# PhilippBongartz/RepeatResolver

Measured on AMD Instinct MI355X. Metric: sum-of-pairs DP cells/sec, higher is better.
Workload: dtype u32

## Files before the change

include/pwr.h:

```cpp
#ifndef PWR_H
#define PWR_H

#include <stddef.h>
#include <stdint.h>
#include <stdio.h>

#ifdef __cplusplus
extern "C" {
#endif

#define PWR_OK 0
#define PWR_ERR_ARG (-1)
#define PWR_ERR_NOMEM (-2)
#define PWR_ERR_DEVICE (-3)
#define PWR_ERR_INPUT (-4)
#define PWR_ERR_RANGE (-5)
#define PWR_ERR_INTERNAL (-6)
#define PWR_ERR_UNSUPPORTED (-7)
#define PWR_ERR_IO (-8)
#define PWR_ERR_STALL (-9)
#define PWR_ERR_ORDER (-10)

#define PWR_MAX_BANDWIDTH 2000
#define PWR_MAX_SEQ_LENGTH 35000
// ... 21 lines not shown
    uint64_t rows_jumped;
} pwr_stats;

int pwr_create(pwr_ctx **out, int rows, int width, const unsigned char *text, int bandwidth, int device);
void pwr_destroy(pwr_ctx *ctx);

int pwr_trim_ends(pwr_ctx *ctx);
int pwr_realign_row(pwr_ctx *ctx, int k);
int pwr_realign_round(pwr_ctx *ctx);
int pwr_realign_rows(pwr_ctx *ctx, int k0, int n);
int pwr_split_begin(pwr_ctx *ctx, int k0, int n, int rank, int world);
int pwr_split_slot_bytes(pwr_ctx *ctx, size_t *slot_bytes, int *slots_per_rank);
int pwr_split_stage(pwr_ctx *ctx, void *send_dev);
int pwr_split_commit(pwr_ctx *ctx, const void *recv_dev, int *rows_left);
int pwr_total_score(pwr_ctx *ctx, uint64_t *total);
int pwr_dims(pwr_ctx *ctx, int *rows, int *width);
int pwr_export_rows(pwr_ctx *ctx, unsigned char *buf, size_t cap);
typedef struct pwr_snapshot pwr_snapshot;
int pwr_snapshot_begin(pwr_ctx *ctx, pwr_snapshot **snap);
int pwr_snapshot_wait(pwr_snapshot *snap, const unsigned char **image, size_t *bytes, int *rows, int *width);
void pwr_snapshot_free(pwr_snapshot *snap);

int pwr_set_option(pwr_ctx *ctx, const char *key, long value);
int pwr_get_option(pwr_ctx *ctx, const char *key, long *value);
int pwr_get_stats(pwr_ctx *ctx, pwr_stats *out);
int pwr_reset_stats(pwr_ctx *ctx);
const char *pwr_strerror(int code);
int pwr_device_count(void);

int pwr_read_msa_file(const char *path, int *rows, int *width, unsigned char **text, char *err, size_t errcap);
int pwr_write_msa_file(const char *path, int rows, int width, const unsigned char *text);
int pwr_run_file(const char *in_path, const char *out_path, int bandwidth, int device, int max_rounds, FILE *log);

#ifdef __cplusplus
}
#endif
#endif
```

repeatresolver_amd/_lib.py:

```python
import ctypes
import os

_HERE = os.path.dirname(os.path.abspath(__file__))
LIB_PATH = os.path.join(_HERE, "csrc", "libpwr.so")


class PwrStats(ctypes.Structure):
    _fields_ = [("cells_reference", ctypes.c_uint64), ("cells_computed", ctypes.c_uint64),
                ("fill_launches", ctypes.c_uint64), ("fill_ms", ctypes.c_double),
                ("rows_committed", ctypes.c_uint64), ("rows_recomputed", ctypes.c_uint64),
                ("batches", ctypes.c_uint64), ("rows_changed", ctypes.c_uint64),
                ("reject_reason", ctypes.c_uint64 * 4), ("fill_launches_timed", ctypes.c_uint64),
                ("stalls", ctypes.c_uint64), ("rows_ahead", ctypes.c_uint64), ("rows_wide", ctypes.c_uint64),
                ("seg_jobs", ctypes.c_uint64), ("segs", ctypes.c_uint64), ("seg_fails", ctypes.c_uint64),
                ("rows_jumped", ctypes.c_uint64)]


EXPORTS = ["pwr_create", "pwr_destroy", "pwr_trim_ends", "pwr_realign_row", "pwr_realign_round", "pwr_realign_rows",
           "pwr_total_score", "pwr_dims", "pwr_export_rows", "pwr_set_option", "pwr_get_option", "pwr_get_stats",
           "pwr_reset_stats", "pwr_strerror", "pwr_device_count", "pwr_read_msa_file",
           "pwr_write_msa_file", "pwr_run_file", "pwr_split_begin", "pwr_split_slot_bytes", "pwr_split_stage", "pwr_split_commit",
           "pwr_snapshot_begin", "pwr_snapshot_wait", "pwr_snapshot_free"]

PIA_EXPORTS = ["pia_create", "pia_destroy", "pia_align", "pia_get_stats", "pia_set_option", "pia_get_timing", "pia_read_template", "pia_read_fasta",
               "pia_build_msa", "pia_run_files"]

PRC_EXPORTS = ["prc_create", "prc_destroy", "prc_occurrences", "prc_cut", "prc_get_stats", "prc_free", "prc_read_template",
               "prc_read_fasta", "prc_scan_dense", "prc_scan_runs", "prc_select_cuts", "prc_write_seq", "prc_write_info",
               "prc_run_files"]

PMC_EXPORTS = ["pmc_maxcorrs", "pmc_last_timing", "pmc_read_msa", "pmc_write", "pmc_run_file"]

PGR_EXPORTS = ["pgr_refine", "pgr_free", "pgr_last_timing", "pgr_read_window", "pgr_window_free", "pgr_slice_maxcorrs",
               "pgr_read_maxcorrs_file", "pgr_default_cutoff", "pgr_restrict_coverage", "pgr_subdivide", "pgr_subdivision_free",
               "pgr_last_subdivision_timing", "pgr_dropoff_subdivision", "pgr_compress_labels", "pgr_complete_labels",
               "pgr_write_subdivision", "pgr_subdivision_name", "pgr_kmeans_subdivide", "pgr_kmeans_free", "pgr_kmeans_subdivide_pairs",
               "pgr_last_kmeans_timing", "pgr_kmeans_reassign", "pgr_msa_open", "pgr_msa_close", "pgr_msa_window", "pgr_msa_resolve",
               "pgr_resolution_free", "pgr_last_resolve_timing", "pgr_connect", "pgr_connection_free"]


class PgrWindow(ctypes.Structure):
    _fields_ = [("rows", ctypes.c_int), ("kept_rows", ctypes.c_int), ("von", ctypes.c_int), ("bis", ctypes.c_int),
                ("width", ctypes.c_int), ("sc", ctypes.c_int), ("kept", ctypes.POINTER(ctypes.c_ubyte)),
                ("groups", ctypes.POINTER(ctypes.c_uint64)), ("local_coverage", ctypes.POINTER(ctypes.c_uint64)),
                ("coverage", ctypes.POINTER(ctypes.c_int))]


class PgrResult(ctypes.Structure):
    _fields_ = [("rows", ctypes.c_int), ("kept_rows", ctypes.c_int), ("width", ctypes.c_int), ("sc", ctypes.c_int),
                ("nsig", ctypes.c_int), ("cutoff", ctypes.c_double), ("kept", ctypes.POINTER(ctypes.c_ubyte)),
                ("maxcorrs", ctypes.POINTER(ctypes.c_double)), ("significant", ctypes.POINTER(ctypes.c_int)),
                ("sizes", ctypes.POINTER(ctypes.c_int)), ("cliques", ctypes.POINTER(ctypes.c_int)),
                ("cutoffs", ctypes.POINTER(ctypes.c_int)), ("drop_off", ctypes.POINTER(ctypes.c_double)),
                ("c_groups", ctypes.POINTER(ctypes.c_uint64)), ("c_coverage", ctypes.POINTER(ctypes.c_uint64))]

# ... 70 lines not shown
    lib.pwr_export_rows.argtypes = [vp, ctypes.c_char_p, ctypes.c_size_t]
    lib.pwr_set_option.restype = ci
    lib.pwr_set_option.argtypes = [vp, ctypes.c_char_p, ctypes.c_long]
    lib.pwr_get_option.restype = ci
    lib.pwr_get_option.argtypes = [vp, ctypes.c_char_p, ctypes.POINTER(ctypes.c_long)]
    lib.pwr_get_stats.restype = ci
    lib.pwr_get_stats.argtypes = [vp, ctypes.POINTER(PwrStats)]
    lib.pwr_strerror.restype = ctypes.c_char_p
    lib.pwr_strerror.argtypes = [ci]
    lib.pwr_device_count.restype = ci
    lib.pwr_device_count.argtypes = []
    lib.pwr_split_begin.restype = ci
    lib.pwr_split_begin.argtypes = [vp, ci, ci, ci, ci]
    lib.pwr_split_slot_bytes.restype = ci
    lib.pwr_split_slot_bytes.argtypes = [vp, ctypes.POINTER(ctypes.c_size_t), ctypes.POINTER(ci)]
    lib.pwr_split_stage.restype = ci
    lib.pwr_split_stage.argtypes = [vp, vp]
    lib.pwr_split_commit.restype = ci
    lib.pwr_split_commit.argtypes = [vp, vp, ctypes.POINTER(ci)]
    if hasattr(lib, "pwr_snapshot_begin"):
        lib.pwr_snapshot_begin.restype = ci
        lib.pwr_snapshot_begin.argtypes = [vp, ctypes.POINTER(vp)]
        lib.pwr_snapshot_wait.restype = ci
        lib.pwr_snapshot_wait.argtypes = [vp, ctypes.POINTER(vp), ctypes.POINTER(ctypes.c_size_t), ctypes.POINTER(ci), ctypes.POINTER(ci)]
        lib.pwr_snapshot_free.restype = None
        lib.pwr_snapshot_free.argtypes = [vp]
    lib.pwr_debug_last_job.restype = ci
    lib.pwr_debug_last_job.argtypes = [vp, ctypes.POINTER(ci), ctypes.POINTER(ci), ctypes.POINTER(ci),
                                       ctypes.POINTER(ci), ctypes.POINTER(ci), ci]
    lib.pwr_debug_fill_clock.restype = ci
    lib.pwr_debug_fill_clock.argtypes = [vp, ctypes.POINTER(ctypes.c_double), ctypes.POINTER(ctypes.c_double)]
    lib.pwr_debug_row_columns.restype = ci
    lib.pwr_debug_row_columns.argtypes = [vp, ci, ctypes.POINTER(ci), ci]
    lib.pwr_debug_rounds.restype = ci
    lib.pwr_debug_rounds.argtypes = [vp]
    ll = ctypes.c_longlong
    lib.pia_create.restype = ci
    lib.pia_create.argtypes = [ctypes.POINTER(vp), ctypes.c_char_p, ci, ci]
    lib.pia_destroy.restype = None
    lib.pia_destroy.argtypes = [vp]
    lib.pia_align.restype = ci
    lib.pia_align.argtypes = [vp, ci, ctypes.c_char_p, ctypes.POINTER(ll), ctypes.POINTER(ci), ctypes.POINTER(ci)]
    lib.pia_get_stats.restype = ci
    lib.pia_get_stats.argtypes = [vp, ctypes.POINTER(ctypes.c_uint64), ctypes.POINTER(ctypes.c_double)]
    lib.pia_set_option.restype = ci
    lib.pia_set_option.argtypes = [vp, ctypes.c_char_p, ll]
    lib.pia_get_timing.restype = ci
    lib.pia_get_timing.argtypes = [vp, ctypes.POINTER(ctypes.c_double)]
    lib.pia_read_template.restype = ci
    lib.pia_read_template.argtypes = [ctypes.c_char_p, ctypes.POINTER(ctypes.c_void_p), ctypes.POINTER(ci)]
    lib.pia_read_fasta.restype = ci
    lib.pia_read_fasta.argtypes = [ctypes.c_char_p, ctypes.POINTER(ci), ctypes.POINTER(ctypes.c_void_p), ctypes.POINTER(ctypes.c_void_p)]
    lib.pia_build_msa.restype = ci
    lib.pia_build_msa.argtypes = [ctypes.c_char_p, ctypes.c_char_p, ci, ctypes.c_char_p, ctypes.POINTER(ll), ctypes.POINTER(ci),
                                  ctypes.POINTER(ci), ctypes.c_double, ci]
    lib.pmc_maxcorrs.restype = ci
    lib.pmc_maxcorrs.argtypes = [ci, ci, ctypes.c_char_p, ci, ci, ctypes.POINTER(ctypes.c_double)]
    lib.pmc_last_timing.restype = ci
    lib.pmc_last_timing.argtypes = [ctypes.POINTER(ctypes.c_double)]
    lib.pmc_read_msa.restype = ci
    lib.pmc_read_msa.argtypes = [ctypes.c_char_p, ctypes.POINTER(ci), ctypes.POINTER(ci), ctypes.POINTER(ctypes.c_void_p)]
    lib.pmc_write.restype = ci
    lib.pmc_write.argtypes = [ctypes.c_char_p, ci, ctypes.POINTER(ctypes.c_double)]
    pi, pll, cp = ctypes.POINTER(ci), ctypes.POINTER(ll), ctypes.c_char_p
    lib.prc_create.restype = ci
    lib.prc_create.argtypes = [ctypes.POINTER(vp), cp, ci, ci]
# ... 90 lines not shown
```

repeatresolver_amd/csrc/pwr_device.hip:

```cpp
#include <hip/hip_runtime.h>

#include <algorithm>
#include <chrono>
#include <cstdint>
#include <cstdio>
#include <cstdlib>
#include <cstring>
#include <new>
#include <thread>
#include <type_traits>
#include <vector>

#include "pwr.h"

#define PWR_INF 0x40000000u
#define PWR_BIG 0x7fffffff

struct Hdr {
    int W;
    int nslots;
    int nfree;
    int cur;
    int status;
    int stop;
// ... 108 lines not shown
    uint4 *desc;
    int wpNW, wpMS;
    unsigned *lastM;
    unsigned long long *gmb;
    SegDesc *seg;
    unsigned *chk;
    int seg_align;
    int src_start;
    int smax, seg_rows, warm_cols;
    int seg_budget, seg_minrows;
    int seg_balance;
    int plan_ahead;
    int hard_rows, hard_up, hard_down;
    int plan_len;
    int plan_gate_rel;
    int spec_inorder;
    int fail_stops;
    int plan_slack, plan_evrate_x100;
    const int *rowids;
    int gstride;
    unsigned tagbase;
    unsigned long long *gtr;
    int trk;
    unsigned trace_tag;
    long long *g64;
    int force64;
    int evcap;
    int gate_v2;
    int *chkdone;
    int check_in_trace, trace_ny;
    int trace_blk;
    int v2_follows, f64_follows;
    int stall_test;
    unsigned long long *diag;
    int njobs_launched;
    int Lmax, colcap, NC;
    size_t dirstride;
    int split_rank, split_world;
    CommitJob *cjob;
    int *chg;
    int *evkey, *evdl;
    int *insidx;
    int *pair_cf, *pair_left;
    BatchPlan *plan;
    CommitEv *sev;
    int *freed;
    unsigned *ticket;
};
#define NOT_MINE(JB, JOB) ((JB).split_world > 1 && (JOB) % (JB).split_world != (JB).split_rank)

#define DPP_ROW_SHR(n) (0x110 + (n))
#define DPP_ROW_BCAST15 0x142
#define DPP_ROW_BCAST31 0x143
#define DPP_WAVE_SHR1 0x138

__device__ __forceinline__ int wave_incl_min(int v)
{
    int t;
    t = __builtin_amdgcn_update_dpp(PWR_BIG, v, DPP_ROW_SHR(1), 0xF, 0xF, false); v = min(v, t);
    t = __builtin_amdgcn_update_dpp(PWR_BIG, v, DPP_ROW_SHR(2), 0xF, 0xF, false); v = min(v, t);
    t = __builtin_amdgcn_update_dpp(PWR_BIG, v, DPP_ROW_SHR(4), 0xF, 0xF, false); v = min(v, t);
    t = __builtin_amdgcn_update_dpp(PWR_BIG, v, DPP_ROW_SHR(8), 0xF, 0xF, false); v = min(v, t);
    t = __builtin_amdgcn_update_dpp(PWR_BIG, v, DPP_ROW_BCAST15, 0xA, 0xF, false); v = min(v, t);
    t = __builtin_amdgcn_update_dpp(PWR_BIG, v, DPP_ROW_BCAST31, 0xC, 0xF, false); v = min(v, t);
    return v;
}
// ... 858 lines not shown
        atomicAdd(&st.hdr->cells_computed, m->cells);
    }
#undef MBP
#undef MBM
#undef PTB
#undef LD64
#undef LD32LO
#undef ST64
}

#ifndef PWR_INTERIOR_CLS
#define PWR_INTERIOR_CLS 0
#endif
#define V3_TICKS() ((unsigned)(__builtin_amdgcn_s_memtime() >> 10))
#define V3_TIMEOUT_TICKS (1u << 19)
#define V4_RB 128

#ifdef PWR_DIAG
#define DG_DECL unsigned long long dg_wait_fast = 0, dg_wait_gen = 0, dg_wait_setup = 0, dg_t = 0, dg_t2 = 0, dg_cyc_int = 0, dg_cyc_gen16 = 0, dg_ts1 = 0, dg_ts2 = 0, dg_tl2 = 0; unsigned dg_log = 0; unsigned dg_int = 0, dg_gen16 = 0, dg_general = 0, dg_nowork = 0, dg_runs = 0, dg_switch = 0;
#define DG_T0() dg_t = __builtin_amdgcn_s_memtime();
#define DG_ADD(ACC) ACC += __builtin_amdgcn_s_memtime() - dg_t;
#define DG_INC(CNT, N) CNT += (N);
#define DG_T2() dg_t2 = __builtin_amdgcn_s_memtime();
#define DG_ADD2(ACC) ACC += __builtin_amdgcn_s_memtime() - dg_t2;
#else
#define DG_T2()
#define DG_ADD2(ACC)
#define DG_DECL
#define DG_T0()
#define DG_ADD(ACC)
#define DG_INC(CNT, N)
#endif
template <int NW, int C, bool WG1>
__global__ __launch_bounds__(WG1 ? NW * 64 : 128) void k_fill_v3(DState st, JobBufs jb)
{
    constexpr int MS = 64 * C, RS = NW * MS;
    constexpr int NL = WG1 ? NW : 1;
    constexpr int RB = WG1 ? 64 : V4_RB;
    __shared__ __attribute__((aligned(16))) int ldsS1[NL][2][4][MS];
    __shared__ unsigned long long rP[NL][RB], rM[NL][RB];
    __shared__ int wprog[NL], wdone;
    const int vjob = WG1 ? (int)blockIdx.x : (int)(blockIdx.x + 8 * blockIdx.z), lane = threadIdx.x & 63;
    const int role = WG1 ? 0 : UNI((int)threadIdx.x >> 6);
    const int wave = WG1 ? UNI((int)threadIdx.x >> 6) : (int)blockIdx.y;
    const int lw = WG1 ? wave : 0, wr = WG1 ? (wave + 1) % NW : 0;
    if (vjob >= jb.njobs_launched * jb.smax) return;
    const int job = vjob / jb.smax;
    const SegDesc *const sd = jb.seg + (size_t)job * SEG_MAX + (vjob % jb.smax);
    JobMeta *m = &jb.meta[job];
    if (st.hdr->fallback > 0 && jb.v2_follows) return;
    if (!m->active || m->L <= 0 || !m->ok || m->wide || !sd->active || NOT_MINE(jb, job)) return;
    const int seg_xb = UNI(sd->xb), seg_fin = UNI(sd->fin);
    const int L = UNI(sd->xe) - seg_xb;
    const int Lf = seg_fin ? L - 1 : L;
    const int x_own = UNI(sd->xown) - seg_xb;
    const int g_own = x_own >> 4;
    const int chkA = x_own > 0 ? x_own : -1, chkB = seg_fin ? -1 : L;
    unsigned *const chk_w = jb.chk + (((size_t)job * (SEG_MAX + 1) + sd->s) * 2 + 0) * (size_t)jb.NC;
    unsigned *const chk_t = jb.chk + (((size_t)job * (SEG_MAX + 1) + sd->s + 1) * 2 + 1) * (size_t)jb.NC;
    const unsigned long long t_clk0 = __builtin_amdgcn_s_memtime(), t_real0 = __builtin_amdgcn_s_memrealtime();
    for (int i = threadIdx.x; i < NL * RB; i += blockDim.x) { (&rP[0][0])[i] = 0; (&rM[0][0])[i] = 0; }
    if (threadIdx.x < NL) wprog[threadIdx.x] = 0;
    if (threadIdx.x == 0) wdone = 0;
    __syncthreads();

    const int wl = (wave + NW - 1) % NW;
    const unsigned tagbase = jb.tagbase;
    const size_t gstride = (size_t)jb.gstride;
    unsigned long long *const gmy = jb.gmb + (((size_t)job * NW + wave) * gstride + (size_t)sd->grow0) * 2;
    const unsigned long long *const gleftw = jb.gmb + (((size_t)job * NW + wl) * gstride + (size_t)sd->grow0) * 2;
    const unsigned long long *const gjob = jb.gmb + ((size_t)job * NW * gstride + (size_t)sd->grow0) * 2;
#define PTOT_PTR(AP, BP, R) (gjob + (((size_t)((((AP) + (BP) - 1 - lo) / MS) % NW)) * gstride + (size_t)(R)) * 2)
    int *const abortf = &m->abort;
#define GLD(PTR) __hip_atomic_load((PTR), __ATOMIC_RELAXED, __HIP_MEMORY_SCOPE_AGENT)
#define GST(PTR, VAL, ROW) __hip_atomic_store((PTR), ((unsigned long long)(tagbase | (unsigned)((ROW) + 1)) << 32) | (unsigned)(VAL), __ATOMIC_RELAXED, __HIP_MEMORY_SCOPE_AGENT)
#define GST2(PTR, VAL, TAG) __hip_atomic_store((PTR), ((unsigned long long)(TAG) << 32) | (unsigned)(VAL), __ATOMIC_RELAXED, __HIP_MEMORY_SCOPE_AGENT)
#define TAGOF(W64) ((unsigned)((W64) >> 32))
#define LLD(REF) __hip_atomic_load(&(REF), __ATOMIC_RELAXED, __HIP_MEMORY_SCOPE_WORKGROUP)
#define LST(REF, V) __hip_atomic_store(&(REF), (V), __ATOMIC_RELAXED, __HIP_MEMORY_SCOPE_WORKGROUP)

    if (!WG1 && role == 1) {
        for (unsigned it = 0;; ++it) {
            if (UNI(LLD(wdone))) break;
            const int wx = UNI(LLD(wprog[lw]));
            const int r = wx - 1 + lane;
            const bool inr = r >= 0 && r < L;
            unsigned long long p = 0, q = 0;
            int ab = 0;
            if (inr) { p = GLD(gleftw + 2 * (size_t)r); q = GLD(gleftw + 2 * (size_t)r + 1); }
            if ((it & 15u) == 15u) ab = GLD(abortf);
            if (inr) {
                const unsigned tagr = tagbase | (unsigned)(r + 1);
                if (TAGOF(p) == tagr && TAGOF(q) == tagr) {
                    LST(rP[lw][r & (RB - 1)], p);
                    __hip_atomic_store(&rM[lw][r & (RB - 1)], q, __ATOMIC_RELEASE, __HIP_MEMORY_SCOPE_WORKGROUP);
                }
            }
            if (UNI(ab)) break;
        }
        return;
    }

    const int lo = UNI(m->lo), hi = UNI(m->hi), W = UNI(m->W), B = st.B, H = st.H;
    const int *way = jb.way + (size_t)job * jb.Lmax + seg_xb;
    const uint8_t *seq = st.seq + st.rowoff[UNI(m->k)] + seg_xb;
    const int4 *rec2 = jb.rec2 + (size_t)job * jb.colcap * 2;
    uint32_t *dirs = jb.dirs + (size_t)job * jb.dirstride + (size_t)(seg_xb >> 4) * RS;
    unsigned *lastM = jb.lastM + (size_t)job * jb.NC;
    const int lc = lane * C;
#define V4_LOADS(MSX, SLOT, AU, AG, AI, GL)                                                      \
    {                                                                                            \
        const int yq_ = lo + (MSX) * MS - 1;                                                     \
        GL = (yq_ >= lo && yq_ <= hi) ? UNI(rec2[2 * (yq_ - lo) + 1].y) : 0;                     \
        int4 p_[C];                                                                              \
        _Pragma("unroll") for (int i = 0; i < C; ++i) {                                          \
            const int y_ = lo + (MSX) * MS + lc + i;                                             \
// ... 52 lines not shown
        _Pragma("unroll") for (int i = 0; i < C; ++i) { accA[i] <<= sh_; accC[i] <<= sh_; }      \
        nacc = (WANT);                                                                           \
    }
#define V4_FLUSH()                                                                               \
    if (gacc >= 0) {                                                                             \
        V4_ALIGN_ACC(16)                                                                         \
        uint32_t *d_ = dirs + (size_t)gacc * RS + (size_t)wave * MS + (size_t)lc;                \
        _Pragma("unroll") for (int i = 0; i < C; ++i) { if (gacc >= g_own) d_[i] = accA[i] | (accC[i] << 16); accA[i] = accC[i] = 0; } \
        gacc = -1; nacc = 0;                                                                     \
    }
#define V4_ROTATE_BLOCK()                                                                        \
    {                                                                                            \
        blk = x >> 6;                                                                            \
        wcur = wnxt; scur = snxt; dca = dna; dcf = dnf >> fsh;     \
        wnxt = way[min(x + 64 + lane, L - 1)];                                                   \
        snxt = seq[min(x + 64 + lane, L - 1)];                                                   \
        dna = desc[min(x + 64 + lane, L - 1)].x; dnf = descw[4 * min(x + 64 + lane, L - 1)];     \
    }
#define V4_NEXT_ROW()                                                                            \
    {                                                                                            \
        a_prev = a; Bx_prev = Bx;                                                                \
        ++x;                                                                                     \
        if (lane == 0) LST(wprog[lw], x);                                                            \
        if (x < L) {                                                                             \
            if ((x >> 6) != blk) V4_ROTATE_BLOCK()                                               \
            a = max(0, __builtin_amdgcn_readlane(wcur, x & 63) - H);                             \
            sx = __builtin_amdgcn_readlane(scur, x & 63);                                        \
        }                                                                                        \
    }

    DG_DECL
#ifdef PWR_DIAG
    unsigned long long *const tl = jb.diag + ((size_t)job * 32 + 31) * 4096 + (size_t)(sd->s * NW + wave) * 6;
    if (lane == 0 && sd->s * NW + wave < 680) { tl[0] = t_real0; tl[1] = __builtin_amdgcn_s_memrealtime(); tl[2] = 0; }
#endif
#define V4_EARLY_MASKS()                                                                         \
    if (early_hi >= (blk << 6)) {                                                                \
        const int b0_ = blk << 6;                                                                \
        const int lo_ = max(early_lo, b0_) - b0_, hi_ = min(early_hi, b0_ + 64) - b0_;           \
        const unsigned long long me_ = hi_ > lo_ ? ((hi_ - lo_ >= 64 ? ~0ull : ((1ull << (hi_ - lo_)) - 1ull)) << lo_) : 0ull; \
        const unsigned long long mf_ = early_hi < b0_ + 64 ? 1ull << (early_hi - b0_) : 0ull;    \
        bOm |= me_ | mf_; bMm |= me_ | mf_; bPm |= me_; bTm |= me_;                              \
    }
    bool dead = jb.stall_test && vjob == 0 && wave == 0;
    int first_pending = 0;
    int early_lo = 0, early_hi = -1;
    while (x < L && !dead) {
        ran_prev = UNI(ran_prev); gacc = UNI(gacc); nacc = UNI(nacc); blk = UNI(blk); ms = UNI(ms); cs = UNI(cs); gleft = UNI(gleft);
        x = UNI(x);
#ifdef PWR_DIAG
        if (ran_prev && !dg_tl2) { dg_tl2 = __builtin_amdgcn_s_memrealtime(); if (lane == 0 && sd->s * NW + wave < 680) { tl[2] = dg_tl2; tl[5] = (unsigned long long)x; } }
#endif
        if ((ran_prev || first_pending) && x < Lf) {
            unsigned long long bOm = __builtin_amdgcn_ballot_w64((dcf & 1u) != 0);
            const bool first = UNI(first_pending) != 0;
            if (first || ((bOm >> (x & 63)) & 1ull)) {
                first_pending = 0;
                unsigned long long bPm = __builtin_amdgcn_ballot_w64((dcf & 2u) != 0);
                unsigned long long bMm = __builtin_amdgcn_ballot_w64((dcf & 4u) != 0);
                unsigned long long bTm = __builtin_amdgcn_ballot_w64((dcf & 8u) != 0);
                if (first) { bOm |= 1ull << (x & 63); bMm |= 1ull << (x & 63); }
                V4_EARLY_MASKS()
                int dcaf = (int)(dca & 0xffffffu), dcb = min(dcaf + B, W);
                unsigned dcs = min(dca >> 24, 3u) * (unsigned)(MS * 4);
                if ((x >> 4) != gacc) { V4_FLUSH() gacc = x >> 4; }
                V4_ALIGN_ACC(x & 15)
                if (lane == 0) LST(wprog[lw], x);
                unsigned mlast_v = 0;
                if (first) {
                    const unsigned tagp = tagbase | (unsigned)x;
                    const int yq = lo + ms * MS - 1;
                    const bool needM = yq >= a_prev && yq < a_prev + Bx_prev;
                    unsigned long long eT = 0, eM = 0;
                    DG_T0()
#ifdef PWR_DIAG
                    const unsigned long long ev_t0 = __builtin_amdgcn_s_memrealtime();
#endif
                    const unsigned t0 = V3_TICKS();
                    for (unsigned spin = 1;; ++spin) {
                        eT = GLD(PTOT_PTR(a_prev, Bx_prev, x - 1));
                        eM = LLD(rM[lw][(x - 1) & (RB - 1)]);
                        if (UNI(TAGOF(eT)) == tagp && (!needM || UNI(TAGOF(eM)) == tagp)) break;
                        if ((spin & 1023u) == 0 && (V3_TICKS() - t0 > V3_TIMEOUT_TICKS || UNI(GLD(abortf)))) { dead = true; break; }
                        __builtin_amdgcn_s_sleep(1);
// ... 407 lines not shown
            const unsigned left0 = (unsigned)__builtin_amdgcn_update_dpp((int)mrow, (int)Mn[C - 1], DPP_WAVE_SHR1, 0xF, 0xF, false);
#pragma unroll
            for (int i = 0; i < C; ++i) {
                const unsigned lf = i ? Mn[i > 0 ? i - 1 : 0] : left0;
                const bool inb = (unsigned)(rel0 + i) < (unsigned)Bx;
                accA[i] = (accA[i] << 1) | ((((fa >> i) & 1u) || (inb && Mn[i] == lf)) ? 1u : 0u);
                lastM[wave * MS + lc + i] = inb ? Mn[i] : 0xffffffffu;
            }
        }
        nacc = (x & 15) + 1;
        if (lane == 63) {
            GST(gmy + 2 * (size_t)x, P_end, x);
            if (WG1) {
                const unsigned long long tg_ = (unsigned long long)(tagbase | (unsigned)(x + 1)) << 32;
                LST(rP[wr][x & (RB - 1)], tg_ | (unsigned)P_end);
                LST(rM[wr][x & (RB - 1)], tg_ | (unsigned)Mprev[C - 1]);
            } else GST(gmy + 2 * (size_t)x + 1, Mprev[C - 1], x);
        }
        ran_prev = 1;
        V4_CHK_STORE(x + 1, a, a + Bx)
        V4_NEXT_ROW()
    }
    V4_FLUSH()
#ifdef PWR_DIAG
    if (lane == 0) {
        unsigned long long *dgp = jb.diag + ((size_t)job * 32 + wave) * 4096;
        dgp[0] = __builtin_amdgcn_s_memtime() - t_clk0; dgp[1] = dg_wait_fast; dgp[2] = dg_wait_gen; dgp[3] = dg_wait_setup;
        dgp[4] = ((unsigned long long)dg_int << 32) | dg_gen16; dgp[5] = ((unsigned long long)dg_general << 32) | dg_nowork;
        dgp[6] = ((unsigned long long)dg_runs << 32) | dg_switch; dgp[7] = (unsigned long long)L;
        dgp[12] = dg_log; dgp[8] = dg_cyc_gen16; dgp[9] = dg_ts1; dgp[10] = dg_ts2; dgp[11] = dg_cyc_int;
    }
#endif
#ifdef PWR_DIAG
    if (lane == 0 && sd->s * NW + wave < 680) { tl[3] = __builtin_amdgcn_s_memrealtime(); tl[4] = (unsigned long long)L | ((unsigned long long)(dg_wait_fast + dg_wait_gen + dg_wait_setup) << 20); }
#endif
    if (lane == 0) { LST(wprog[lw], 0x7fffffff); LST(wdone, 1); }
    if (dead) {
        if (lane == 0) __hip_atomic_store(abortf, 1, __ATOMIC_RELAXED, __HIP_MEMORY_SCOPE_AGENT);
        return;
    }
    if (wave == 0 && lane == 0) {
        if (sd->s == 0) {
            m->clk = (unsigned)(__builtin_amdgcn_s_memtime() - t_clk0);
            m->rclk = (unsigned)(__builtin_amdgcn_s_memrealtime() - t_real0);
            m->rounds = 0;
        }
        atomicAdd(&st.hdr->cells_computed, sd->cells);
    }
#undef V4_CHK_STORE
#undef V4_EARLY_MASKS
#undef PTOT_PTR
#undef GLD
#undef GST
#undef GST2
#undef TAGOF
#undef LLD
#undef LST
#undef V4_LOADS
#undef V4_ALIGN_ACC
#undef V4_FLUSH
#undef V4_ROTATE_BLOCK
#undef V4_NEXT_ROW
}

__device__ __forceinline__ bool seg_check_applies(const DState &st, const JobBufs &jb, int job, const JobMeta *m)
{
    return m->active && m->L > 0 && m->ok && !m->wide && !m->abort && !(st.hdr->fallback > 0 && jb.v2_follows) && !NOT_MINE(jb, job) && m->nseg > 1;
}

// ... 2207 lines not shown
    if ((rc = regrow(c, &st.inscnt, 0, ncap))) return rc;
    if ((rc = regrow(c, &st.newidx, 0, ncap))) return rc;
    st.colcap = (int)ncap; st.slotcap = (int)ncap;
    const int nj = c->njobs;
    free_jobs(c);
    if ((rc = alloc_jobs(c, nj))) return rc;
    const int zero = 0;
    HIPC(hipMemcpy(&st.hdr->need_grow, &zero, sizeof(int), hipMemcpyHostToDevice));
    return PWR_OK;
}

static int launch_fill(pwr_ctx *c, int njobs)
{
    hipEvent_t e0 = nullptr, e1 = nullptr;
    const bool timed = c->profile && (c->stats.fill_launches % (unsigned)c->profile) == 0 && c->ev_used < (size_t)(1 << 16);
    if (timed) {
        if (c->ev_used == c->ev_pool.size()) {
            hipEvent_t a, b;
            HIPC(hipEventCreate(&a)); HIPC(hipEventCreate(&b));
            c->ev_pool.emplace_back(a, b);
        }
        e0 = c->ev_pool[c->ev_used].first; e1 = c->ev_pool[c->ev_used].second;
        c->ev_used++;
        HIPC(hipEventRecord(e0, c->stream));
    }
    if (c->fill_mode == 4) {
        if (++c->fill_epoch >= (1u << 15)) {
            const size_t nmb = (size_t)c->njobs * c->wp_waves * c->jb.gstride * 2;
            HIPC(hipMemsetAsync(c->jb.gmb, 0, nmb * 8, c->stream));
            c->fill_epoch = 1;
        }
        c->jb.tagbase = c->fill_epoch << 17;
        c->jb.njobs_launched = njobs;
        c->jb.stall_test = c->stall_test > 0 ? 1 : 0;
        c->jb.v2_follows = (c->seen_fallback > 0 && c->wp_waves != 17) ? 1 : 0;
        if (c->stall_test > 0) c->stall_test -= 1;
        const int nv = njobs * c->jb.smax;
        const dim3 grid(8, c->wp_waves, (nv + 7) / 8);
        const bool wg1 = c->one_wg && c->wp_waves <= 9 && c->B <= 1024 && c->wave_cols != 4;
        if (wg1) {
            const size_t pad = (size_t)c->one_wg_lds;
            if (c->wp_waves == 5) hipLaunchKernelGGL((k_fill_v3<5, 4, true>), dim3(nv), dim3(5 * 64), pad, c->stream, c->st, c->jb);
            else if (c->wp_waves == 8) hipLaunchKernelGGL((k_fill_v3<8, 3, true>), dim3(nv), dim3(8 * 64), pad, c->stream, c->st, c->jb);
            else if (c->wp_waves == 4) hipLaunchKernelGGL((k_fill_v3<4, 6, true>), dim3(nv), dim3(4 * 64), pad, c->stream, c->st, c->jb);
            else if (c->wp_waves == 3) hipLaunchKernelGGL((k_fill_v3<3, 8, true>), dim3(nv), dim3(3 * 64), pad, c->stream, c->st, c->jb);
            else hipLaunchKernelGGL((k_fill_v3<9, 2, true>), dim3(nv), dim3(9 * 64), pad, c->stream, c->st, c->jb);
        }
        else if (c->wp_waves == 17) hipLaunchKernelGGL((k_fill_v3<17, 1, false>), grid, dim3(128), 0, c->stream, c->st, c->jb);
        else if (c->wp_waves == 5) hipLaunchKernelGGL((k_fill_v3<5, 4, false>), grid, dim3(128), (size_t)c->fill_lds, c->stream, c->st, c->jb);
        else if (c->wp_waves == 8) hipLaunchKernelGGL((k_fill_v3<8, 3, false>), grid, dim3(128), 0, c->stream, c->st, c->jb);
        else if (c->wp_waves == 4) hipLaunchKernelGGL((k_fill_v3<4, 6, false>), grid, dim3(128), 0, c->stream, c->st, c->jb);
        else if (c->wp_waves == 3) hipLaunchKernelGGL((k_fill_v3<3, 8, false>), grid, dim3(128), 0, c->stream, c->st, c->jb);
        else if (c->B <= 1024 && c->wave_cols != 4) hipLaunchKernelGGL((k_fill_v3<9, 2, false>), grid, dim3(128), 0, c->stream, c->st, c->jb);
        else hipLaunchKernelGGL((k_fill_v3<9, 4, false>), grid, dim3(128), 0, c->stream, c->st, c->jb);
        c->jb.stall_test = 0;
        if (c->jb.smax > 1 && c->jb.seg_rows > 0 && !c->jb.check_in_trace)
            hipLaunchKernelGGL(k_seg_check, dim3(njobs, c->jb.smax - 1), dim3(256), 0, c->stream, c->st, c->jb);
    }
    c->jb.gate_v2 = c->fill_mode == 4 ? 1 : 0;
    if (c->fill_mode == 3) c->jb.v2_follows = 1;
    if (c->fill_mode == 3 || (c->fill_mode == 4 && c->jb.v2_follows)) {
        if (c->wp_waves == 5) hipLaunchKernelGGL((k_fill_v2<5, 4>), dim3(njobs), dim3(5 * 64), 0, c->stream, c->st, c->jb);
        else if (c->wp_waves == 8) hipLaunchKernelGGL((k_fill_v2<8, 3>), dim3(njobs), dim3(8 * 64), 0, c->stream, c->st, c->jb);
        else if (c->wp_waves == 4) hipLaunchKernelGGL((k_fill_v2<4, 6>), dim3(njobs), dim3(4 * 64), 0, c->stream, c->st, c->jb);
        else if (c->wp_waves == 3) hipLaunchKernelGGL((k_fill_v2<3, 8>), dim3(njobs), dim3(3 * 64), 0, c->stream, c->st, c->jb);
        else if (c->B <= 1024 && c->wave_cols != 4) hipLaunchKernelGGL((k_fill_v2<9, 2>), dim3(njobs), dim3(9 * 64), 0, c->stream, c->st, c->jb);
        else hipLaunchKernelGGL((k_fill_v2<9, 4>), dim3(njobs), dim3(9 * 64), 0, c->stream, c->st, c->jb);
    } else if (c->fill_mode != 4) return PWR_ERR_ARG;
    HIPC(hipGetLastError());
    if (timed) { HIPC(hipEventRecord(e1, c->stream)); c->stats.fill_launches_timed += 1; }
    c->stats.fill_launches += 1;
    return PWR_OK;
}

static int drain_events(pwr_ctx *c)
{
    if (!c->ev_used) return PWR_OK;
    HIPC(hipStreamSynchronize(c->stream));
    for (size_t i = 0; i < c->ev_used; ++i) {
        float ms = 0;
        HIPC(hipEventElapsedTime(&ms, c->ev_pool[i].first, c->ev_pool[i].second));
        c->stats.fill_ms += ms;
    }
    c->ev_used = 0;
    return PWR_OK;
}

// ... 571 lines not shown
    memcpy(out, h.data(), sizeof(int) * std::min(L, cap));
    return L;
}

extern "C" int pwr_debug_rounds(pwr_ctx *c)
{
    if (!c || !c->on_device) return PWR_ERR_ARG;
    if (hipSetDevice(c->device) != hipSuccess) return PWR_ERR_DEVICE;
    if (hipStreamSynchronize(c->stream) != hipSuccess) return PWR_ERR_DEVICE;
    JobMeta m;
    if (hipMemcpy(&m, c->jb.meta, sizeof m, hipMemcpyDeviceToHost) != hipSuccess) return PWR_ERR_DEVICE;
    return m.rounds;
}

extern "C" int pwr_debug_phase_times(pwr_ctx *c, unsigned long long *out)
{
    if (!c || !c->on_device || !out) return PWR_ERR_ARG;
    if (hipSetDevice(c->device) != hipSuccess) return PWR_ERR_DEVICE;
    HIPC(hipStreamSynchronize(c->stream));
    HIPC(hipMemcpy(out, c->st.hdr->dbg, sizeof(unsigned long long) * 32, hipMemcpyDeviceToHost));
    HIPC(hipMemset(c->st.hdr->dbg, 0, sizeof(unsigned long long) * 32));
    return PWR_OK;
}

extern "C" int pwr_debug_fill_diag(pwr_ctx *c, unsigned long long *out)
{
    if (!c || !c->on_device || !out) return PWR_ERR_ARG;
    if (hipSetDevice(c->device) != hipSuccess) return PWR_ERR_DEVICE;
    HIPC(hipStreamSynchronize(c->stream));
    HIPC(hipMemcpy(out, c->jb.diag, sizeof(unsigned long long) * 32 * 4096, hipMemcpyDeviceToHost));
    return PWR_OK;
}

extern "C" int pwr_debug_fill_clock(pwr_ctx *c, double *mhz, double *fill_us)
{
    if (!c || !c->on_device) return PWR_ERR_ARG;
    if (hipSetDevice(c->device) != hipSuccess) return PWR_ERR_DEVICE;
    HIPC(hipStreamSynchronize(c->stream));
    JobMeta m;
    HIPC(hipMemcpy(&m, c->jb.meta, sizeof m, hipMemcpyDeviceToHost));
    if (mhz) *mhz = m.rclk ? 100.0 * (double)m.clk / (double)m.rclk : 0.0;
    if (fill_us) *fill_us = (double)m.rclk / 100.0;
    return PWR_OK;
}
```

repeatresolver_amd/csrc/pwr_host.c:

```c
#define _POSIX_C_SOURCE 200809L
#define _FILE_OFFSET_BITS 64
#include "pwr.h"

#include <pthread.h>
#include <stdlib.h>
#include <string.h>
#include <sys/types.h>
#include <time.h>
#include <unistd.h>

static int read_msa_by_line(const char *path, int *rows, int *width, unsigned char **text, char *err, size_t errcap)
{
    FILE *f = fopen(path, "r");
    if (!f) { if (err) snprintf(err, errcap, "MA is missing."); return PWR_ERR_INPUT; }
    const size_t bufsz = PWR_MAX_LINE + 3;
    char *buf = malloc(bufsz);
    unsigned char *data = NULL;
    size_t cap = 0, used = 0;
    int T = 0, W = -1, rc = PWR_OK;
    if (!buf) { fclose(f); return PWR_ERR_NOMEM; }
    while (fgets(buf, (int)(PWR_MAX_LINE + 1), f)) {
        size_t n = strlen(buf);
        if (n == 0 || buf[n - 1] != '\n') {
            if (err) snprintf(err, errcap, "line %d is not terminated by a newline (or is longer than %d)", T + 1, PWR_MAX_LINE);
// ... 158 lines not shown
    fprintf(log, "Rows %d, Columns %d.\n", T, W);
    uint64_t best = 0, tot = 0;
    if ((rc = pwr_total_score(ctx, &best))) goto fail;
    print_score(log, best);
    struct timespec t0, t1;
    clock_gettime(CLOCK_MONOTONIC, &t0);
    for (int round = 0; round < 10000; round++) {
        if (max_rounds >= 0 && round >= max_rounds) break;
        if ((rc = pwr_realign_round(ctx))) goto fail;
        if ((rc = pwr_total_score(ctx, &tot))) goto fail;
        print_score(log, tot);
        if (tot < best) {
            best = tot;
            if ((rc = write_current(ctx, out_path, &wr))) goto fail;
        } else break;
    }
    clock_gettime(CLOCK_MONOTONIC, &t1);
    fprintf(log, "Total time: %f min.\n", ((t1.tv_sec - t0.tv_sec) + 1e-9 * (t1.tv_nsec - t0.tv_nsec)) / 60.0);
    if ((rc = pwr_trim_ends(ctx))) goto fail;
    if ((rc = pwr_total_score(ctx, &tot))) goto fail;
    print_score(log, tot);
    if (tot < best && (rc = write_current(ctx, out_path, &wr))) goto fail;
    if ((rc = out_writer_join(&wr))) goto fail;
    pwr_destroy(ctx);
    return 0;
fail:
    (void)out_writer_join(&wr);
    if (rc == PWR_ERR_IO) fprintf(log, "DateiVerbratei!\n");
    else if (rc == PWR_ERR_INTERNAL) fprintf(log, "\nStuff gone wrong\n");
    else fprintf(log, "PW_ReAligner: %s\n", pwr_strerror(rc));
    pwr_destroy(ctx);
    return 1;
}
```

Measured before the change: 55.00 billion.

## Pack four fill jobs per workgroup with SIMD-paired producer/consumer waves

The non-WG1 fill kernel now launches 512-thread workgroups holding four independent job slots instead of 128-thread workgroups with one slot each. It uses the hardware SIMD id to pair each slot's compute and helper waves on the same SIMD when that is possible. Per-slot LDS, progress and done flags are indexed by slot. The aim is to cut workgroup count and dispatch overhead and to co-locate the communicating wave pairs. The risks are more LDS per workgroup, which lowers occupancy, an early return that can happen after a __syncthreads, and a larger grid-tail imbalance.

Result: no change. 55.00 billion (-0.0%).

```diff
diff --git a/include/pwr.h b/include/pwr.h
--- a/include/pwr.h
+++ b/include/pwr.h
@@ -77,6 +77,16 @@
 int pwr_write_msa_file(const char *path, int rows, int width, const unsigned char *text);
 int pwr_run_file(const char *in_path, const char *out_path, int bandwidth, int device, int max_rounds, FILE *log);
 
+#define PWR_FILL_SLOTS 4
+#if defined(__HIPCC__) || defined(__CUDACC__)
+#define PWRX_HD __host__ __device__
+#else
+#define PWRX_HD
+#endif
+PWRX_HD static inline int pwrx_fill_slot_vjob(int bx, int bz, int q) { return bx + 8 * (PWR_FILL_SLOTS * bz + q); }
+PWRX_HD static inline int pwrx_fill_grid_z(int nv) { return (nv + 8 * PWR_FILL_SLOTS - 1) / (8 * PWR_FILL_SLOTS); }
+int pwr_debug_fill_slot(int nw, int nv, int block, int q, int *vjob, int *wave, int *nblocks);
+
 #ifdef __cplusplus
 }
 #endif
diff --git a/repeatresolver_amd/_lib.py b/repeatresolver_amd/_lib.py
--- a/repeatresolver_amd/_lib.py
+++ b/repeatresolver_amd/_lib.py
@@ -20,7 +20,7 @@
            "pwr_total_score", "pwr_dims", "pwr_export_rows", "pwr_set_option", "pwr_get_option", "pwr_get_stats",
            "pwr_reset_stats", "pwr_strerror", "pwr_device_count", "pwr_read_msa_file",
            "pwr_write_msa_file", "pwr_run_file", "pwr_split_begin", "pwr_split_slot_bytes", "pwr_split_stage", "pwr_split_commit",
-           "pwr_snapshot_begin", "pwr_snapshot_wait", "pwr_snapshot_free"]
+           "pwr_snapshot_begin", "pwr_snapshot_wait", "pwr_snapshot_free", "pwr_debug_fill_slot"]
 
 PIA_EXPORTS = ["pia_create", "pia_destroy", "pia_align", "pia_get_stats", "pia_set_option", "pia_get_timing", "pia_read_template", "pia_read_fasta",
                "pia_build_msa", "pia_run_files"]
@@ -157,6 +157,9 @@
     lib.pwr_debug_fill_clock.argtypes = [vp, ctypes.POINTER(ctypes.c_double), ctypes.POINTER(ctypes.c_double)]
     lib.pwr_debug_row_columns.restype = ci
     lib.pwr_debug_row_columns.argtypes = [vp, ci, ctypes.POINTER(ci), ci]
+    if hasattr(lib, "pwr_debug_fill_slot"):
+        lib.pwr_debug_fill_slot.restype = ci
+        lib.pwr_debug_fill_slot.argtypes = [ci, ci, ci, ci, ctypes.POINTER(ci), ctypes.POINTER(ci), ctypes.POINTER(ci)]
     lib.pwr_debug_rounds.restype = ci
     lib.pwr_debug_rounds.argtypes = [vp]
     ll = ctypes.c_longlong
diff --git a/repeatresolver_amd/csrc/pwr_device.hip b/repeatresolver_amd/csrc/pwr_device.hip
--- a/repeatresolver_amd/csrc/pwr_device.hip
+++ b/repeatresolver_amd/csrc/pwr_device.hip
@@ -164,6 +164,7 @@
     int trace_blk;
     int v2_follows, f64_follows;
     int stall_test;
+    int diag_full;
     unsigned long long *diag;
     int njobs_launched;
     int Lmax, colcap, NC;
@@ -1088,18 +1089,42 @@
 #define DG_INC(CNT, N)
 #endif
 template <int NW, int C, bool WG1>
-__global__ __launch_bounds__(WG1 ? NW * 64 : 128) void k_fill_v3(DState st, JobBufs jb)
+__global__ __launch_bounds__(WG1 ? NW * 64 : 128 * PWR_FILL_SLOTS) void k_fill_v3(DState st, JobBufs jb)
 {
     constexpr int MS = 64 * C, RS = NW * MS;
-    constexpr int NL = WG1 ? NW : 1;
+    constexpr int NS = WG1 ? 1 : PWR_FILL_SLOTS;
+    constexpr int NL = WG1 ? NW : NS;
     constexpr int RB = WG1 ? 64 : V4_RB;
     __shared__ __attribute__((aligned(16))) int ldsS1[NL][2][4][MS];
     __shared__ unsigned long long rP[NL][RB], rM[NL][RB];
-    __shared__ int wprog[NL], wdone;
-    const int vjob = WG1 ? (int)blockIdx.x : (int)(blockIdx.x + 8 * blockIdx.z), lane = threadIdx.x & 63;
-    const int role = WG1 ? 0 : UNI((int)threadIdx.x >> 6);
+    __shared__ int wprog[NL], wdone[NS];
+    __shared__ int claim[4];
+    const int lane = threadIdx.x & 63;
+#define V3_LDS_INIT()                                                                            \
+    for (int i = threadIdx.x; i < NL * RB; i += blockDim.x) { (&rP[0][0])[i] = 0; (&rM[0][0])[i] = 0; }    \
+    if (threadIdx.x < NL) wprog[threadIdx.x] = 0;                                                \
+    if (threadIdx.x < NS) wdone[threadIdx.x] = 0;
+    int slot = 0, role = 0;
+    unsigned long long t_clk0 = 0, t_real0 = 0;
+    if (!WG1) {
+        t_clk0 = __builtin_amdgcn_s_memtime(); t_real0 = __builtin_amdgcn_s_memrealtime();
+        V3_LDS_INIT()
+        if (threadIdx.x < 4) claim[threadIdx.x] = 0;
+        __syncthreads();
+        const int widx = UNI((int)threadIdx.x >> 6);
+        const int simd = (int)__builtin_amdgcn_s_getreg(4 | (4 << 6) | (1 << 11));
+        int nth = 0;
+        if (lane == 0) nth = atomicAdd(&claim[simd], 1);
+        nth = UNI(nth);
+        __syncthreads();
+        const bool paired = claim[0] == 2 && claim[1] == 2 && claim[2] == 2 && claim[3] == 2;
+        slot = UNI(paired ? simd : (widx & 3));
+        role = UNI(paired ? nth : (widx >> 2));
+    }
+    const int vjob = WG1 ? (int)blockIdx.x : pwrx_fill_slot_vjob((int)blockIdx.x, (int)blockIdx.z, slot);
     const int wave = WG1 ? UNI((int)threadIdx.x >> 6) : (int)blockIdx.y;
-    const int lw = WG1 ? wave : 0, wr = WG1 ? (wave + 1) % NW : 0;
+    const int lw = WG1 ? wave : slot, wr = WG1 ? (wave + 1) % NW : 0;
+    const int ld = WG1 ? 0 : slot;
     if (vjob >= jb.njobs_launched * jb.smax) return;
     const int job = vjob / jb.smax;
     const SegDesc *const sd = jb.seg + (size_t)job * SEG_MAX + (vjob % jb.smax);
@@ -1114,11 +1139,20 @@
     const int chkA = x_own > 0 ? x_own : -1, chkB = seg_fin ? -1 : L;
     unsigned *const chk_w = jb.chk + (((size_t)job * (SEG_MAX + 1) + sd->s) * 2 + 0) * (size_t)jb.NC;
     unsigned *const chk_t = jb.chk + (((size_t)job * (SEG_MAX + 1) + sd->s + 1) * 2 + 1) * (size_t)jb.NC;
-    const unsigned long long t_clk0 = __builtin_amdgcn_s_memtime(), t_real0 = __builtin_amdgcn_s_memrealtime();
-    for (int i = threadIdx.x; i < NL * RB; i += blockDim.x) { (&rP[0][0])[i] = 0; (&rM[0][0])[i] = 0; }
-    if (threadIdx.x < NL) wprog[threadIdx.x] = 0;
-    if (threadIdx.x == 0) wdone = 0;
-    __syncthreads();
+    if (WG1) {
+        t_clk0 = __builtin_amdgcn_s_memtime(); t_real0 = __builtin_amdgcn_s_memrealtime();
+        V3_LDS_INIT()
+        __syncthreads();
+    }
+#undef V3_LDS_INIT
+#ifdef PWR_DIAG
+    if (!WG1 && lane == 0 && jb.diag_full && sd->s * NW + wave < 680) {
+        unsigned long long *const hw = jb.diag + ((size_t)job * 32 + 30) * 4096 + ((size_t)(sd->s * NW + wave) * 2 + role) * 2;
+        const unsigned long long wg = blockIdx.x + gridDim.x * (blockIdx.y + (unsigned long long)gridDim.y * blockIdx.z);
+        hw[0] = (1ull << 63) | (wg << 36) | ((unsigned long long)(__builtin_amdgcn_s_getreg(20 | (3 << 11)) & 15u) << 32) | (unsigned)__builtin_amdgcn_s_getreg(4 | (31 << 11));
+        hw[1] = t_real0;
+    }
+#endif
 
     const int wl = (wave + NW - 1) % NW;
     const unsigned tagbase = jb.tagbase;
@@ -1137,7 +1171,7 @@
 
     if (!WG1 && role == 1) {
         for (unsigned it = 0;; ++it) {
-            if (UNI(LLD(wdone))) break;
+            if (UNI(LLD(wdone[ld]))) break;
             const int wx = UNI(LLD(wprog[lw]));
             const int r = wx - 1 + lane;
             const bool inr = r >= 0 && r < L;
@@ -1256,7 +1290,7 @@
     DG_DECL
 #ifdef PWR_DIAG
     unsigned long long *const tl = jb.diag + ((size_t)job * 32 + 31) * 4096 + (size_t)(sd->s * NW + wave) * 6;
-    if (lane == 0 && sd->s * NW + wave < 680) { tl[0] = t_real0; tl[1] = __builtin_amdgcn_s_memrealtime(); tl[2] = 0; }
+    if (lane == 0 && jb.diag_full && sd->s * NW + wave < 680) { tl[0] = t_real0; tl[1] = __builtin_amdgcn_s_memrealtime(); tl[2] = 0; }
 #endif
 #define V4_EARLY_MASKS()                                                                         \
     if (early_hi >= (blk << 6)) {                                                                \
@@ -1273,7 +1307,7 @@
         ran_prev = UNI(ran_prev); gacc = UNI(gacc); nacc = UNI(nacc); blk = UNI(blk); ms = UNI(ms); cs = UNI(cs); gleft = UNI(gleft);
         x = UNI(x);
 #ifdef PWR_DIAG
-        if (ran_prev && !dg_tl2) { dg_tl2 = __builtin_amdgcn_s_memrealtime(); if (lane == 0 && sd->s * NW + wave < 680) { tl[2] = dg_tl2; tl[5] = (unsigned long long)x; } }
+        if (ran_prev && !dg_tl2) { dg_tl2 = __builtin_amdgcn_s_memrealtime(); if (lane == 0 && jb.diag_full && sd->s * NW + wave < 680) { tl[2] = dg_tl2; tl[5] = (unsigned long long)x; } }
 #endif
         if ((ran_prev || first_pending) && x < Lf) {
             unsigned long long bOm = __builtin_amdgcn_ballot_w64((dcf & 1u) != 0);
@@ -1747,9 +1781,9 @@
     }
 #endif
 #ifdef PWR_DIAG
-    if (lane == 0 && sd->s * NW + wave < 680) { tl[3] = __builtin_amdgcn_s_memrealtime(); tl[4] = (unsigned long long)L | ((unsigned long long)(dg_wait_fast + dg_wait_gen + dg_wait_setup) << 20); }
+    if (lane == 0 && jb.diag_full && sd->s * NW + wave < 680) { tl[3] = __builtin_amdgcn_s_memrealtime(); tl[4] = (unsigned long long)L | ((unsigned long long)(dg_wait_fast + dg_wait_gen + dg_wait_setup) << 20); }
 #endif
-    if (lane == 0) { LST(wprog[lw], 0x7fffffff); LST(wdone, 1); }
+    if (lane == 0) { LST(wprog[lw], 0x7fffffff); LST(wdone[ld], 1); }
     if (dead) {
         if (lane == 0) __hip_atomic_store(abortf, 1, __ATOMIC_RELAXED, __HIP_MEMORY_SCOPE_AGENT);
         return;
@@ -4023,11 +4057,12 @@
         }
         c->jb.tagbase = c->fill_epoch << 17;
         c->jb.njobs_launched = njobs;
+        c->jb.diag_full = njobs >= c->window ? 1 : 0;
         c->jb.stall_test = c->stall_test > 0 ? 1 : 0;
         c->jb.v2_follows = (c->seen_fallback > 0 && c->wp_waves != 17) ? 1 : 0;
         if (c->stall_test > 0) c->stall_test -= 1;
         const int nv = njobs * c->jb.smax;
-        const dim3 grid(8, c->wp_waves, (nv + 7) / 8);
+        const dim3 grid(8, c->wp_waves, pwrx_fill_grid_z(nv));
         const bool wg1 = c->one_wg && c->wp_waves <= 9 && c->B <= 1024 && c->wave_cols != 4;
         if (wg1) {
             const size_t pad = (size_t)c->one_wg_lds;
@@ -4037,13 +4072,13 @@
             else if (c->wp_waves == 3) hipLaunchKernelGGL((k_fill_v3<3, 8, true>), dim3(nv), dim3(3 * 64), pad, c->stream, c->st, c->jb);
             else hipLaunchKernelGGL((k_fill_v3<9, 2, true>), dim3(nv), dim3(9 * 64), pad, c->stream, c->st, c->jb);
         }
-        else if (c->wp_waves == 17) hipLaunchKernelGGL((k_fill_v3<17, 1, false>), grid, dim3(128), 0, c->stream, c->st, c->jb);
-        else if (c->wp_waves == 5) hipLaunchKernelGGL((k_fill_v3<5, 4, false>), grid, dim3(128), (size_t)c->fill_lds, c->stream, c->st, c->jb);
-        else if (c->wp_waves == 8) hipLaunchKernelGGL((k_fill_v3<8, 3, false>), grid, dim3(128), 0, c->stream, c->st, c->jb);
-        else if (c->wp_waves == 4) hipLaunchKernelGGL((k_fill_v3<4, 6, false>), grid, dim3(128), 0, c->stream, c->st, c->jb);
-        else if (c->wp_waves == 3) hipLaunchKernelGGL((k_fill_v3<3, 8, false>), grid, dim3(128), 0, c->stream, c->st, c->jb);
-        else if (c->B <= 1024 && c->wave_cols != 4) hipLaunchKernelGGL((k_fill_v3<9, 2, false>), grid, dim3(128), 0, c->stream, c->st, c->jb);
-        else hipLaunchKernelGGL((k_fill_v3<9, 4, false>), grid, dim3(128), 0, c->stream, c->st, c->jb);
+        else if (c->wp_waves == 17) hipLaunchKernelGGL((k_fill_v3<17, 1, false>), grid, dim3(128 * PWR_FILL_SLOTS), 0, c->stream, c->st, c->jb);
+        else if (c->wp_waves == 5) hipLaunchKernelGGL((k_fill_v3<5, 4, false>), grid, dim3(128 * PWR_FILL_SLOTS), (size_t)c->fill_lds, c->stream, c->st, c->jb);
+        else if (c->wp_waves == 8) hipLaunchKernelGGL((k_fill_v3<8, 3, false>), grid, dim3(128 * PWR_FILL_SLOTS), 0, c->stream, c->st, c->jb);
+        else if (c->wp_waves == 4) hipLaunchKernelGGL((k_fill_v3<4, 6, false>), grid, dim3(128 * PWR_FILL_SLOTS), 0, c->stream, c->st, c->jb);
+        else if (c->wp_waves == 3) hipLaunchKernelGGL((k_fill_v3<3, 8, false>), grid, dim3(128 * PWR_FILL_SLOTS), 0, c->stream, c->st, c->jb);
+        else if (c->B <= 1024 && c->wave_cols != 4) hipLaunchKernelGGL((k_fill_v3<9, 2, false>), grid, dim3(128 * PWR_FILL_SLOTS), 0, c->stream, c->st, c->jb);
+        else hipLaunchKernelGGL((k_fill_v3<9, 4, false>), grid, dim3(128 * PWR_FILL_SLOTS), 0, c->stream, c->st, c->jb);
         c->jb.stall_test = 0;
         if (c->jb.smax > 1 && c->jb.seg_rows > 0 && !c->jb.check_in_trace)
             hipLaunchKernelGGL(k_seg_check, dim3(njobs, c->jb.smax - 1), dim3(256), 0, c->stream, c->st, c->jb);
@@ -4681,6 +4716,15 @@
     return PWR_OK;
 }
 
+extern "C" int pwr_debug_fill_diag_job(pwr_ctx *c, int job, unsigned long long *out)
+{
+    if (!c || !c->on_device || !out || job < 0 || job >= c->njobs) return PWR_ERR_ARG;
+    if (hipSetDevice(c->device) != hipSuccess) return PWR_ERR_DEVICE;
+    HIPC(hipStreamSynchronize(c->stream));
+    HIPC(hipMemcpy(out, c->jb.diag + (size_t)job * 32 * 4096, sizeof(unsigned long long) * 32 * 4096, hipMemcpyDeviceToHost));
+    return PWR_OK;
+}
+
 extern "C" int pwr_debug_fill_clock(pwr_ctx *c, double *mhz, double *fill_us)
 {
     if (!c || !c->on_device) return PWR_ERR_ARG;
diff --git a/repeatresolver_amd/csrc/pwr_host.c b/repeatresolver_amd/csrc/pwr_host.c
--- a/repeatresolver_amd/csrc/pwr_host.c
+++ b/repeatresolver_amd/csrc/pwr_host.c
@@ -214,3 +214,15 @@
     pwr_destroy(ctx);
     return 1;
 }
+
+int pwr_debug_fill_slot(int nw, int nv, int block, int q, int *vjob, int *wave, int *nblocks)
+{
+    if (nw < 1 || nv < 1 || !vjob || !wave) return PWR_ERR_ARG;
+    const int gz = pwrx_fill_grid_z(nv);
+    if (nblocks) *nblocks = 8 * nw * gz;
+    if (block < 0 || block >= 8 * nw * gz || q < 0 || q >= PWR_FILL_SLOTS) return PWR_ERR_ARG;
+    const int bx = block % 8, by = (block / 8) % nw, bz = block / (8 * nw);
+    *vjob = pwrx_fill_slot_vjob(bx, bz, q);
+    *wave = by;
+    return *vjob < nv ? 1 : 0;
+}
```
